# wizardyesterday/RtlSdrDiags

Measured on AMD Instinct MI355X. Metric: IQ MSamples/s through WBFM chain at 1/2/4/8 GPUs; % HBM roofline, higher is better.
Workload: dtype int8/int16 Q15 + f32; 1 GPU; BASELINE configs[1]: WBFM, 1 channel, 2^28-sample synthetic IQ; channels_per_gpu=1, log2_samples_per_channel=28, kernels=streaming pipelines

## Files before the change

rtlsdrdiags_amd/csrc/iqd_stream.hip:

```cpp
#include <hip/hip_runtime.h>

#include "iqd_kernels.h"
#include "iqd_stream.h"
#include "iqd_wbfm.h"
#include "iqd_mfma.h"
#include "iqd_stream_fix.h"
#include "iqd_taps.h"

namespace iqd {

#define ST_STORE16(P, A, B, C, D) (*(u32x4 *)(P) = u32x4{A, B, C, D})


typedef __attribute__((address_space(3))) const uint32_t lds_cu32;
__device__ __forceinline__ uint32_t st_table_read(uint32_t byte_offset) { return *(lds_cu32 *)(uintptr_t)byte_offset; }

#ifndef IQD_ST_WAITSTAT
#define IQD_ST_WAITSTAT 0
#endif

#ifndef IQD_ST_SLEEP_P
#define IQD_ST_SLEEP_P 6
#endif
#ifndef IQD_ST_SLEEP_I
#define IQD_ST_SLEEP_I 10
#endif
#ifndef IQD_ST_SLEEP_A
#define IQD_ST_SLEEP_A 10
#endif
#define ST_TAP(WHICH, Q) (uint32_t)taps::STREAM_TAPS.WHICH[Q]
#ifndef IQD_ST_TRACE
#define IQD_ST_TRACE 0
#endif
#if IQD_ST_TRACE
#define ST_TRACE(st, wave, piece, k) do { if (blockIdx.x == 5 && lane == 0 && (piece) < 256) (st)[64 + (((wave) * 256 + (int)(piece)) * 4 + (k))] = (unsigned long long)clock64(); } while (0)
#else
#define ST_TRACE(st, wave, piece, k) do { } while (0)
#endif
#ifndef IQD_ST_TIMING
#define IQD_ST_TIMING 0
#endif
#if IQD_ST_TIMING
#define ST_T(var) const long long var = clock64()
__device__ __forceinline__ int st_simd_id() { return (__builtin_amdgcn_s_getreg((4 << 0) | (4 << 6) | (1 << 11)) ) & 3; }
#else
#define ST_T(var) do { } while (0)
#endif

template <int ROT, bool MAG, bool EPOCHS, bool GATED, bool BYGROUP = false>
__device__ __forceinline__ void st_p_wave(const ChainLaunch &a, const StreamArgs &sa, uint8_t *lds, uint32_t *sync,
                                          int pw, int lane, uint32_t &pc)
{
    const int cg = pw / ST_RINGS, ring = pw % ST_RINGS;
    if (ring >= (int)sa.rings) return;
    const uint32_t wg_segs = 64u * sa.rings;
    const int g = lane >> 4, c = lane & 15;
    const uint32_t row = (uint32_t)(16 * cg + c);
    uint8_t *ring_base = lds + ST_TABLE_BYTES + ring * (ST_RING_SLOTS * ST_SLOT_BYTES);
    const uint32_t *full = sync + ring * 8;
    asm volatile("" : "+v"(full));
    const uint32_t *consumed = full + 4;
    const uint32_t wr_off = st_slot_off(row, (uint32_t)g);
    const int src_lane4 = ((lane - 16) & 63) << 2;

    v4i A[8];
#pragma unroll
    for (int m = 0; m < 8; m++) A[m] = ((const v4i *)(BYGROUP ? sa.amat3[1 - ROT] : sa.amat))[m * 64 + lane];
    v4i cbias = {WB_BIAS, WB_BIAS, WB_BIAS, WB_BIAS};
    const v4i czero = {0, 0, 0, 0};
    asm volatile("" : "+v"(cbias));
    uint32_t zero = 0;
    asm volatile("" : "+v"(zero));

    const int n_pieces = (ST_HALO + (int)a.tile_len) >> 5;
    uint64_t inv_2pi = 0x3e22f9843e22f984ull;
    asm volatile("" : "+s"(inv_2pi));
    for (uint32_t round = 0; round < sa.rounds; round++) {
        if ((round * chain_wgs(a) + chain_wg(a)) * wg_segs >= st_id_count(sa)) break;
        const uint32_t sid = (round * chain_wgs(a) + chain_wg(a)) * wg_segs + ring * 64 + row;
        int rot_of_id = ROT;
        const StSeg sg = BYGROUP ? st_segment_of(a, sa, sid, rot_of_id) : st_segment(a, sid, sa.n_segments);
        if (BYGROUP && __builtin_amdgcn_readfirstlane(rot_of_id) != ROT) continue;
        const ChanParams &p = a.params[sg.ech];
        const uint8_t *iq_ch = a.iq + (size_t)sg.ch * a.ch_stride_bytes;
        const uint8_t *tail = a.tails + ((size_t)sg.ech * FAM_COUNT + FAM_WBFM) * TAIL_BYTES + TAIL_BYTES;
        const int32_t vmax = sg.vlen - 8;
        const float kneg = -p.wbfm_k;
        const GainEpochList *ep = &a.epochs[sg.ech].wbfm;
        const bool ep_reach = EPOCHS && ep->since[0] < (uint32_t)TAIL && (int64_t)sg.v0 - ST_HALO - 32 < -(int64_t)ep->since[0];
        const bool ep_any = EPOCHS && __any(ep_reach);
        const int32_t mlim = MAG && sg.valid ? sg.tlen : INT32_MIN;
        uint32_t macc = 0;
        const uint32_t mblk0 = (uint32_t)sg.v0 / a.block_samples;
        uint32_t minblk = (uint32_t)sg.v0 - mblk0 * a.block_samples;
        uint32_t *mag_at = MAG ? a.mag_sums + (size_t)sg.ch * a.n_blocks + mblk0 : nullptr;
        uint32_t gm16 = 0;

        const int32_t vlane = sg.v0 + 8 * g;
        const uint8_t *base_iq = iq_ch + 2 * (int64_t)vlane, *base_tail = tail + 2 * (int64_t)vlane;
        const int32_t pos_max = vmax - vlane;
        const uint32_t *blk_list = GATED ? a.blk_lists + (size_t)sg.ch * a.n_blocks : nullptr;
        int32_t gb_v0 = 0, gb_v1 = 0;
        const uint8_t *gb_base = iq_ch;
        auto piece_address = [&](int pos) -> const uint8_t * {
            const int32_t pc = pos < pos_max ? pos : pos_max;
            if (!GATED) {
                const uint8_t *base = pc < -vlane ? base_tail : base_iq;
                return base + 2 * (int64_t)pc;
            }
            const int32_t vv = vlane + pc;
            if (vv >= 0 && (vv >= gb_v1 || vv < gb_v0)) {
                const uint32_t blk = (uint32_t)vv / a.block_samples;
                gb_v0 = (int32_t)(blk * a.block_samples);
                gb_v1 = gb_v0 + (int32_t)a.block_samples;
                gb_base = iq_ch + 2 * ((int64_t)blk_list[blk] * a.block_samples - (int64_t)gb_v0);
            }
            return vv < 0 ? base_tail + 2 * (int64_t)pc : gb_base + 2 * (int64_t)vv;
        };
        const int32_t pos_last = pos_max & ~31;
        const bool from_tail = sg.v0 == 0;
        const uint8_t *nxt = piece_address(-ST_HALO + 32 * ST_AHEAD);
        uint4 prev = st_front<ROT>(*(const uint4 *)piece_address(-ST_HALO - 32), zero);
        v4u raw[ST_AHEAD];
#pragma unroll
        for (int j = 0; j < ST_AHEAD; j++) raw[j] = gload16_untracked(piece_address(-ST_HALO + 32 * j));
        float last_prev;
        {
            const v4i bn = v4i{(int)prev.x, (int)prev.y, (int)prev.z, (int)prev.w};
            const v4i ilo = __builtin_amdgcn_mfma_i32_16x16x64_i8(A[0], bn, cbias, 0, 0, 0);
            const v4i ihi = __builtin_amdgcn_mfma_i32_16x16x64_i8(A[1], bn, czero, 0, 0, 0);
            const v4i qlo = __builtin_amdgcn_mfma_i32_16x16x64_i8(A[2], bn, cbias, 0, 0, 0);
            const v4i qhi = __builtin_amdgcn_mfma_i32_16x16x64_i8(A[3], bn, czero, 0, 0, 0);
            const uint32_t ti = (uint32_t)ilo[3] + ((uint32_t)ihi[3] << 8), tq = (uint32_t)qlo[3] + ((uint32_t)qhi[3] << 8);
            asm volatile("" :: "v"(ilo), "v"(ihi), "v"(qlo), "v"(qhi), "v"(ti), "v"(tq));
            uint32_t rr;
            asm("v_msad_u8 %0, %1, %2, 0" : "=v"(rr) : "v"(tq), "s"(0x00800000u));
            const uint32_t t = st_table_read(rr * (uint32_t)(ST_ROW_FLOATS * 4) + (bfe(ti, 16, 8) << 2));
            last_prev = u2f((t & 0x7fffffffu) | ((tq << 8) & 0x80000000u));
        }
        uint32_t n_sleeps = 0;
#if IQD_ST_TIMING
        long long tt[4] = {0, 0, 0, 0};
#endif
        auto do_piece = [&](const int q, const int j, const uint4 &prev, uint4 &cur) __attribute__((always_inline)) {
            const int pos = -ST_HALO + 32 * q;
            ST_TRACE(a.stamps, pw + 3, q, 0);
            ST_T(t0);
            gload_wait<ST_AHEAD - 1>(raw[j]);
            ST_T(t1);
            const uint4 raw_cur = as_uint4(raw[j]);
            cur = st_front<ROT>(raw_cur, zero);
            const v4i bs = v4i{(int)(lane < 32 ? cur.x : prev.x), (int)(lane < 32 ? cur.y : prev.y),
                               (int)(lane < 32 ? cur.z : prev.z), (int)(lane < 32 ? cur.w : prev.w)};
            const v4i bn = v4i{(int)cur.x, (int)cur.y, (int)cur.z, (int)cur.w};
            v4i acc[2][4];
            acc[0][0] = __builtin_amdgcn_mfma_i32_16x16x64_i8(A[4], bs, cbias, 0, 0, 0);
            acc[0][1] = __builtin_amdgcn_mfma_i32_16x16x64_i8(A[5], bs, czero, 0, 0, 0);
            acc[0][2] = __builtin_amdgcn_mfma_i32_16x16x64_i8(A[6], bs, cbias, 0, 0, 0);
            acc[0][3] = __builtin_amdgcn_mfma_i32_16x16x64_i8(A[7], bs, czero, 0, 0, 0);
            acc[1][0] = __builtin_amdgcn_mfma_i32_16x16x64_i8(A[0], bn, cbias, 0, 0, 0);
            acc[1][1] = __builtin_amdgcn_mfma_i32_16x16x64_i8(A[1], bn, czero, 0, 0, 0);
            acc[1][2] = __builtin_amdgcn_mfma_i32_16x16x64_i8(A[2], bn, cbias, 0, 0, 0);
            acc[1][3] = __builtin_amdgcn_mfma_i32_16x16x64_i8(A[3], bn, czero, 0, 0, 0);
            uint32_t traw[2][4], tqs[2][4];
#pragma unroll
            for (int half = 0; half < 2; half++) {
#pragma unroll
                for (int r = 0; r < 4; r++) {
                    const uint32_t ti = (uint32_t)acc[half][0][r] + ((uint32_t)acc[half][1][r] << 8);
                    const uint32_t tq = (uint32_t)acc[half][2][r] + ((uint32_t)acc[half][3][r] << 8);
                    uint32_t rr;
                    asm("v_msad_u8 %0, %1, %2, 0" : "=v"(rr) : "v"(tq), "s"(0x00800000u));
                    const uint32_t x4 = bfe(ti, 16, 8) << 2;
                    uint32_t addr;
                    asm("v_mad_u32_u24 %0, %1, %2, %3" : "=v"(addr) : "v"(rr), "s"((uint32_t)(ST_ROW_FLOATS * 4)), "v"(x4));
                    traw[half][r] = st_table_read(addr);
                    tqs[half][r] = tq;
                }
            }
            uint32_t seen = lds_load_relaxed(consumed);
            if (MAG && pos >= 0) gm16 = st_mag_raw_chunk(raw_cur, gm16);
            if (GATED) {
                raw[j] = gload16_untracked(piece_address(pos + 32 * ST_AHEAD));
            } else {
                raw[j] = gload16_untracked(nxt);
                nxt += pos + 32 * ST_AHEAD < pos_last ? 64 : 0;
            }
            float u[2][4];
#pragma unroll
            for (int half = 0; half < 2; half++) {
                const int wpos = pos + 16 * half;
                float th[4];
#pragma unroll
                for (int r = 0; r < 4; r++) {
                    uint32_t bits;
                    asm("v_bfi_b32 %0, %1, %2, %3" : "=v"(bits) : "s"(0x7fffffffu), "v"(traw[half][r]), "v"(tqs[half][r] << 8));
                    th[r] = u2f(bits);
                }
                const float give = g == 3 ? last_prev : th[3];
                const float before = u2f((uint32_t)__builtin_amdgcn_ds_bpermute(src_lane4, (int)f2u(give)));
                last_prev = th[3];
                float kk = kneg;
                if (EPOCHS && ep_any && ep_reach) kk = -epoch_gain_search(ep, p.wbfm_k, sg.v0 + wpos);
#pragma unroll
                for (int r = 0; r < 4; r += 2) {
                    v2f d = {th[r] - (r == 0 ? before : th[r - 1]), th[r + 1] - th[r]};
                    v2f m = pk_mul_s(d, inv_2pi);
                    m.x = __builtin_rintf(m.x);
                    m.y = __builtin_rintf(m.y);
                    d = __builtin_elementwise_fma(-m, v2f{6.28318548202514648f, 6.28318548202514648f}, d);
                    d = __builtin_elementwise_fma(-m, v2f{-1.74845553146951715e-7f, -1.74845553146951715e-7f}, d);
                    const v2f v = d * v2f{kk, kk};
                    const v2f w = v2f{sa.b0, sa.b0} * v;
                    u[half][r] = w.x;
                    u[half][r + 1] = w.y;
                }
            }
            ST_T(t2);
            ST_TRACE(a.stamps, pw + 3, q, 1);
            while ((int32_t)(seen + (uint32_t)(ST_DEPTH - 1) - pc) < 0) {
                __builtin_amdgcn_s_sleep(IQD_ST_SLEEP_P);
                seen = lds_load_relaxed(consumed);
                if (IQD_ST_WAITSTAT) n_sleeps++;
            }
            ST_T(t3);
            ST_TRACE(a.stamps, pw + 3, q, 2);
            __builtin_amdgcn_fence(__ATOMIC_ACQUIRE, "workgroup");
            uint8_t *const slot = ring_base + (ST_DEPTH > 1 ? (pc & (uint32_t)(ST_DEPTH - 1)) * (2 * ST_SLOT_BYTES) : 0u) + wr_off;
            *(u32x4 *)slot = u32x4{f2u(u[0][0]), f2u(u[0][1]), f2u(u[0][2]), f2u(u[0][3])};
            *(u32x4 *)(slot + ST_SLOT_BYTES) = u32x4{f2u(u[1][0]), f2u(u[1][1]), f2u(u[1][2]), f2u(u[1][3])};
            __builtin_amdgcn_fence(__ATOMIC_RELEASE, "workgroup");
            lds_signal(ST_DEPTH > 1 ? full + (pc & (uint32_t)(ST_DEPTH - 1)) : full);
            ST_TRACE(a.stamps, pw + 3, q, 3);
            pc++;
#if IQD_ST_TIMING
            { ST_T(t4); tt[0] += t1 - t0; tt[1] += t2 - t1; tt[2] += t3 - t2; tt[3] += t4 - t3; }
#endif
        };
        uint4 other;
        for (int q = 0; q < n_pieces; q += ST_AHEAD) {
#pragma unroll
            for (int j = 0; j < ST_AHEAD; j += 2) {
                do_piece(q + j, j, prev, other);
                do_piece(q + j + 1, j + 1, other, prev);
            }
            const int gpos = -ST_HALO + 32 * q;
            if (!GATED && gpos + 64 * ST_AHEAD == 0)
                nxt = from_tail ? a.iq + (size_t)sg.ch * a.ch_stride_bytes + 16 * g : nxt;
            if (MAG && gpos >= 0) {
                const uint32_t m = (gm16 & 0xffffu) + (gm16 >> 16);
                gm16 = 0;
                macc += gpos < mlim ? m : 0u;
                minblk += 32 * ST_AHEAD;
                if (minblk >= a.block_samples) {
                    if (macc) atomicAdd(mag_at, macc);
                    macc = 0;
                    mag_at++;
                    minblk -= a.block_samples;
                }
            }
        }
#pragma unroll
        for (int j = 0; j < ST_AHEAD; j++) gload_wait<0>(raw[j]);
        if (MAG && macc) atomicAdd(mag_at, macc);
        if (IQD_ST_WAITSTAT && lane == 0) {
            atomicAdd(&a.stamps[0], (unsigned long long)n_sleeps);
            atomicAdd(&a.stamps[2], (unsigned long long)n_pieces);
        }
#if IQD_ST_TIMING
        if (lane == 0) {
            atomicAdd(&a.stamps[16 + pw], (unsigned long long)tt[1]);
            atomicAdd(&a.stamps[32 + pw], (unsigned long long)tt[2]);
            atomicAdd(&a.stamps[48 + pw], (unsigned long long)(tt[0] + tt[3]));
        }
#endif
    }
}

struct StIir {
    float y, up;
    uint32_t wlast[2];
    uint32_t wq0[2];
    uint32_t y1h[4];
    uint32_t y2lo;
    uint32_t n_sleeps;
    int ring;
    unsigned long long *stamps;
#if IQD_ST_TIMING
    long long t_wait, t_seen, t_to_consumed;
#endif
};

__device__ __forceinline__ int st_iir_window(const StreamArgs &sa, StIir &s, const float (&u)[16], int c14, int c15)
{
    uint32_t wq[10];
    float y = s.y, up = s.up;
    const float a1 = sa.a1;
#pragma unroll
    for (int k = 0; k < 8; k++) {
        IQD_IIR_STEP(u[2 * k])
        const float y_even = y;
        IQD_IIR_STEP(u[2 * k + 1])
        wq[2 + k] = cast_pack_i16_bounded(y_even, y);
    }
    s.y = y;
    s.up = up;
    wq[0] = s.wlast[0];
    wq[1] = s.wlast[1];
    s.wlast[0] = wq[8];
    s.wlast[1] = wq[9];
    s.wq0[0] = wq[2];
    s.wq0[1] = wq[3];
    uint32_t y1[4];
#pragma unroll
    for (int o = 0; o < 4; o++) {
        int acc = dot2_from(wq[2 * o], sa.d1p2[0], c15);
        acc = dot2(wq[2 * o + 1], ST_TAP(d1p2, 1), acc);
        acc = dot2(wq[2 * o + 2], ST_TAP(d1p2, 2), acc);
        acc = dot2(wq[2 * o + 3], ST_TAP(d1p2, 3), acc);
        y1[o] = (uint32_t)acc;
    }
    const uint32_t d[6] = {s.y1h[0], s.y1h[1], s.y1h[2], s.y1h[3], pack_hi16(y1[0], y1[1]), pack_hi16(y1[2], y1[3])};
    int acc = dot2_from(d[5], sa.p12p[0], c14);
#pragma unroll
    for (int q = 1; q < 6; q++) acc = dot2(d[5 - q], ST_TAP(p12p, q), acc);
    s.y1h[0] = d[2];
    s.y1h[1] = d[3];
    s.y1h[2] = d[4];
    s.y1h[3] = d[5];
    return acc >> 15;
}

struct StIirSeg {
    StSeg sg;
    int32_t back;
    float cy_y, cy_u;
    int32_t rec_pos;
    WbfmRecord rec;
    StHist *hist;
    int c14, c15;
};

__device__ __forceinline__ bool st_ring_is_fast(uint32_t valid, int32_t back, int32_t tlen, uint32_t tile_len, bool keeps_restart)
{
    return __all(!valid || (back < 0 && tlen == (int32_t)tile_len && !keeps_restart)) != 0;
}

struct StY2Ring {
    uint8_t *lane_slot0;
    const uint32_t *full, *consumed;
};
__device__ __forceinline__ StY2Ring st_y2_ring(uint8_t *lds, uint32_t *sync, int ring, int lane)
{
    return StY2Ring{lds + ST_Y2_OFF + ring * ST_Y2_RING_BYTES + lane * 4, sync + ring * 8 + ST_SYNC_Y2_FULL, sync + ring * 8 + ST_SYNC_Y2_CONSUMED};
}

__device__ __forceinline__ void st_iir_marks(const ChainLaunch &a, StIirSeg &q, StIir &s, int pos, int rec_pos_uniform)
{
    if (q.back >= 0) {
        if (pos == -q.back) { s.y = q.cy_y; s.up = q.cy_u; }
        else if (pos < -q.back) { s.y = 0.f; s.up = 0.f; }
    } else if (pos == 0) {
        q.rec.y_in = s.y;
    }
    if (pos == q.rec_pos) {
        if (q.sg.valid & 2u) {
            q.hist->pad[0] = f2u(s.y);
            q.hist->pad[1] = f2u(s.up);
        } else {
            q.rec.y_out = s.y;
            q.rec.u_out = s.up;
        }
    }
    if ((q.sg.valid & 2u) && pos == rec_pos_uniform) { q.rec.y_out = s.y; q.rec.u_out = s.up; }
    if (pos == q.sg.tlen) {
        q.rec.y_end = s.y;
        q.rec.u_end = s.up;
        if (q.sg.valid) {
            ST_STORE16(q.hist->y1_last, s.y1h[0], s.y1h[1], s.y1h[2], s.y1h[3]);
            *(u32x2 *)q.hist->w_last = u32x2{s.wlast[0], s.wlast[1]};
        }
    }
}

template <bool FAST>
__device__ __forceinline__ void st_iir_piece(const ChainLaunch &a, const StreamArgs &sa, uint8_t *ring_base, const uint32_t *full, uint32_t *consumed,
                                             uint32_t &wg, const StY2Ring &y2r, uint32_t &yk, StIirSeg &q, StIir &s, int pos, uint32_t rd_off0,
                                             uint32_t rd_swz, int lane, int rec_pos_uniform)
{
    uint32_t y2_seen = 0;
#pragma unroll
    for (int half = 0; half < 2; half++) {
        const int wpos = pos + 16 * half;
        if (half == 0) {
            const uint32_t target = 4u * (wg / (uint32_t)ST_DEPTH + 1u);
            const uint32_t *const fullp = ST_DEPTH > 1 ? full + (wg & (uint32_t)(ST_DEPTH - 1)) : full;
            ST_T(tw0);
            while ((int32_t)(lds_load_relaxed(fullp) - target) < 0) {
                __builtin_amdgcn_s_sleep(IQD_ST_SLEEP_I);
                if (IQD_ST_WAITSTAT) s.n_sleeps++;
            }
#if IQD_ST_TIMING
            { ST_T(tw1); s.t_wait += tw1 - tw0; s.t_seen = tw1; }
#endif
            ST_TRACE(s.stamps, s.ring, wg, 0);
            __builtin_amdgcn_fence(__ATOMIC_ACQUIRE, "workgroup");
        }
        const uint8_t *slot = ring_base + (ST_DEPTH > 1 ? (wg & (uint32_t)(ST_DEPTH - 1)) * (2 * ST_SLOT_BYTES) : 0u) + half * ST_SLOT_BYTES + rd_off0;
        float u[16];
#pragma unroll
        for (int gq = 0; gq < 4; gq++) {
            const u32x4 v = *(const u32x4 *)(slot + (((uint32_t)gq ^ rd_swz) << 4));
            u[4 * gq] = u2f(v.x); u[4 * gq + 1] = u2f(v.y); u[4 * gq + 2] = u2f(v.z); u[4 * gq + 3] = u2f(v.w);
        }
        if (half == 1) {
            y2_seen = lds_load_relaxed(y2r.consumed);
            __builtin_amdgcn_fence(__ATOMIC_RELEASE, "workgroup");
            lds_signal(consumed);
            ST_TRACE(s.stamps, s.ring, wg, 1);
            wg++;
#if IQD_ST_TIMING
            { ST_T(tc); s.t_to_consumed += tc - s.t_seen; }
#endif
        }
        if (!FAST) st_iir_marks(a, q, s, wpos, rec_pos_uniform);
        else if (wpos == rec_pos_uniform) { q.rec.y_out = s.y; q.rec.u_out = s.up; }
        const int y2 = st_iir_window(sa, s, u, q.c14, q.c15);
        if (wpos >= 0 && wpos < 48 && q.sg.valid) {
            if (wpos == 0) ST_STORE16(q.hist->w_first, s.wq0[0], s.wq0[1], s.y1h[2], s.y1h[3]);
            else *(u32x2 *)&q.hist->y1_first[wpos >> 3] = u32x2{s.y1h[2], s.y1h[3]};
        }
        if (half == 0) s.y2lo = (uint32_t)y2;
        else {
            const StY2Piece yp = st_y2_piece(yk, ST_Y2_DEPTH, ST_Y2_EVERY);
            while ((int32_t)(y2_seen - yp.need_consumed) < 0) {
                __builtin_amdgcn_s_sleep(IQD_ST_SLEEP_I);
                y2_seen = lds_load_relaxed(y2r.consumed);
                if (IQD_ST_WAITSTAT) s.n_sleeps++;
            }
            __builtin_amdgcn_fence(__ATOMIC_ACQUIRE, "workgroup");
            *(uint32_t *)(y2r.lane_slot0 + yp.slot * ST_Y2_SLOT_BYTES) = pack_lo16(s.y2lo, (uint32_t)y2);
            __builtin_amdgcn_fence(__ATOMIC_RELEASE, "workgroup");
            if (yp.add_full) lds_signal(y2r.full, yp.add_full);
            yk++;
        }
    }
    ST_TRACE(s.stamps, s.ring, wg - 1, 2);
}

__device__ __forceinline__ void st_iir_lead_in(const StreamArgs &sa, uint8_t *ring_base, const uint32_t *full, uint32_t *consumed,
                                               uint32_t &wg, StIir &s, uint32_t rd_off0, uint32_t rd_swz)
{
    float y = s.y, up = s.up;
    const float a1 = sa.a1;
    for (int piece = 0; piece < ST_HALO / 32; piece++) {
        const uint32_t target = 4u * (wg / (uint32_t)ST_DEPTH + 1u);
        while ((int32_t)(lds_load_relaxed(ST_DEPTH > 1 ? full + (wg & (uint32_t)(ST_DEPTH - 1)) : full) - target) < 0) __builtin_amdgcn_s_sleep(IQD_ST_SLEEP_I);
        __builtin_amdgcn_fence(__ATOMIC_ACQUIRE, "workgroup");
        u32x4 v[8];
#pragma unroll
        for (int half = 0; half < 2; half++)
#pragma unroll
            for (int gq = 0; gq < 4; gq++)
                v[4 * half + gq] = *(const u32x4 *)(ring_base + (ST_DEPTH > 1 ? (wg & (uint32_t)(ST_DEPTH - 1)) * (2 * ST_SLOT_BYTES) : 0u) +
                                                    half * ST_SLOT_BYTES + rd_off0 + (((uint32_t)gq ^ rd_swz) << 4));
        __builtin_amdgcn_fence(__ATOMIC_RELEASE, "workgroup");
        lds_signal(consumed);
        wg++;
#pragma unroll
        for (int k = 0; k < 8; k++) {
            IQD_IIR_STEP(u2f(v[k].x)) IQD_IIR_STEP(u2f(v[k].y)) IQD_IIR_STEP(u2f(v[k].z)) IQD_IIR_STEP(u2f(v[k].w))
        }
    }
    s.y = y;
    s.up = up;
}

__device__ __forceinline__ void st_iir_wave(const ChainLaunch &a, const StreamArgs &sa, uint8_t *lds, uint32_t *sync,
                                            int ring, int lane)
{
    uint8_t *ring_base = lds + ST_TABLE_BYTES + ring * (ST_RING_SLOTS * ST_SLOT_BYTES);
    const uint32_t *full = sync + ring * 8;
    uint32_t *consumed = sync + ring * 8 + 4;
    const StY2Ring y2r = st_y2_ring(lds, sync, ring, lane);
    const uint32_t rd_off0 = (uint32_t)lane * 64u, rd_swz = ((uint32_t)lane >> 2) & 3u;
    const int n_pieces = (ST_HALO + (int)a.tile_len) >> 5;
    if (ring >= (int)sa.rings) return;
    const uint32_t wg_segs = 64u * sa.rings;
    uint32_t wg = 0;
    uint32_t yk = 0;
    for (uint32_t round = 0; round < sa.rounds; round++) {
        if ((round * chain_wgs(a) + chain_wg(a)) * wg_segs >= st_id_count(sa)) break;
        const uint32_t sid = (round * chain_wgs(a) + chain_wg(a)) * wg_segs + ring * 64 + lane;
        StIirSeg q;
        int rot_unused;
        q.sg = st_segment_of(a, sa, sid, rot_unused);
        q.hist = sa.hist + (q.sg.valid ? (size_t)q.sg.li * a.tiles_per_ch + q.sg.tile : 0);
        q.back = -1;
        q.cy_y = q.cy_u = 0.f;
        q.c14 = 1 << 14;
        q.c15 = 1 << 15;
        asm volatile("" : "+v"(q.c14), "+v"(q.c15));
        int32_t carried_back = ST_HALO;
        if (q.sg.tile == 0) {
            const WbfmCarry cy = a.wbfm_carry[q.sg.ech];
            q.back = cy.back;
            q.cy_y = cy.y;
            q.cy_u = cy.u;
            carried_back = cy.back;
        }
        const StRecPlan rp = st_rec_plan(q.sg.valid, q.sg.tile, q.sg.v0, q.sg.tlen, q.sg.vlen, carried_back);
        q.rec_pos = rp.park_pos;
        q.rec.y_in = q.cy_y;
        q.rec.y_out = q.cy_y;
        q.rec.u_out = q.cy_u;
        q.rec.back_out = rp.back_out;
        q.rec.y_end = 0.f;
        q.rec.u_end = 0.f;
        q.rec.pad[0] = q.rec.pad[1] = 0;
        const bool keeps_restart = rp.keeps_restart != 0;
        StIir s;
        s.y = 0.f; s.up = 0.f;
        s.wlast[0] = s.wlast[1] = 0;
        s.wq0[0] = s.wq0[1] = 0;
#pragma unroll
        for (int k = 0; k < 4; k++) s.y1h[k] = 0;
        s.y2lo = 0;
        s.n_sleeps = 0;
        s.ring = ring;
        s.stamps = a.stamps;
#if IQD_ST_TIMING
        s.t_wait = 0;
        s.t_seen = 0;
        s.t_to_consumed = 0;
        const long long t_iir0 = clock64();
#endif
        const bool fast = st_ring_is_fast(q.sg.valid, q.back, q.sg.tlen, a.tile_len, keeps_restart);
        if (keeps_restart) q.sg.valid |= 2u;
        const int rec_pos_uniform = (int)a.tile_len - FORCED_BACK;
        if (fast) {
            st_iir_lead_in(sa, ring_base, full, consumed, wg, s, rd_off0, rd_swz);
            q.rec.y_in = s.y;
            for (int pq = ST_HALO / 32; pq < n_pieces; pq++)
                st_iir_piece<true>(a, sa, ring_base, full, consumed, wg, y2r, yk, q, s, -ST_HALO + 32 * pq, rd_off0, rd_swz, lane, rec_pos_uniform);
        } else {
            for (int pq = 0; pq < n_pieces; pq++)
                st_iir_piece<false>(a, sa, ring_base, full, consumed, wg, y2r, yk, q, s, -ST_HALO + 32 * pq, rd_off0, rd_swz, lane, rec_pos_uniform);
        }
        st_iir_marks(a, q, s, (int)a.tile_len, rec_pos_uniform);
        if (q.sg.valid) {
            WbfmRecord *const r = a.records + (size_t)q.sg.li * a.tiles_per_ch + q.sg.tile;
            if (q.sg.valid & 2u) {
                q.rec.pad[0] = q.hist->pad[0];
                q.rec.pad[1] = q.hist->pad[1];
            } else if (!(q.sg.vlen - q.sg.v0 > q.sg.tlen)) {
                q.rec.pad[0] = WBFM_REC_STREAMED;
            }
            *r = q.rec;
        }
        if (IQD_ST_WAITSTAT && lane == 0) {
            atomicAdd(&a.stamps[1], (unsigned long long)s.n_sleeps);
            atomicAdd(&a.stamps[3], (unsigned long long)n_pieces);
        }
#if IQD_ST_TIMING
        if (lane == 0) {
            atomicAdd(&a.stamps[28 + ring], (unsigned long long)s.t_wait);
            atomicAdd(&a.stamps[44 + ring], (unsigned long long)(clock64() - t_iir0));
            atomicAdd(&a.stamps[60 + ring], (unsigned long long)s.t_to_consumed);
        }
#endif
    }
}

template <int V>
__device__ __forceinline__ int st_audio(const StreamArgs &sa, const uint32_t (&y2p)[24], bool quiet, int c14)
{
    int acc = c14;
    if (quiet) {
        acc = dot2_from(y2p[V + 20], sa.a40p[0], c14);
#pragma unroll
        for (int q = 1; q < 20; q++) acc = dot2(y2p[V + 20 - q], ST_TAP(a40p, q), acc);
    } else {
#pragma unroll
        for (int q = 0; q < 20; q++) {
            acc = clamp_q30(dot2(y2p[V + 20 - q], ST_TAP(a40p, q) & 0xffff0000u, acc));
            acc = clamp_q30(dot2(y2p[V + 20 - q], ST_TAP(a40p, q) & 0x0000ffffu, acc));
        }
    }
    return acc >> 15;
}

struct StAudRing {
    uint32_t y2p[24];
    uint32_t pbuf[2];
    int16_t *pcm;
    uint32_t hidx;
    int32_t tlen;
};

template <int V>
__device__ __forceinline__ uint32_t st_audio_piece(const StreamArgs &sa, const StY2Ring &y2r, uint32_t &ak, StAudRing &r, int &loud, int c14)
{
    const StY2Piece yp = st_y2_piece(ak, ST_Y2_DEPTH, ST_Y2_EVERY);
    while ((int32_t)(lds_load_relaxed(y2r.full) - yp.need_full) < 0) __builtin_amdgcn_s_sleep(IQD_ST_SLEEP_A);
    __builtin_amdgcn_fence(__ATOMIC_ACQUIRE, "workgroup");
    const uint32_t pair = *(const uint32_t *)(y2r.lane_slot0 + yp.slot * ST_Y2_SLOT_BYTES);
    __builtin_amdgcn_fence(__ATOMIC_RELEASE, "workgroup");
    lds_signal(y2r.consumed);
    ak++;
    r.y2p[V + 20] = pair;
    const int lo = (int)(pair << 16) >> 16, hi = (int)pair >> 16;
    const uint32_t mlo = (uint32_t)(lo < 0 ? -lo : lo), mhi = (uint32_t)(hi < 0 ? -hi : hi);
    if (__any(mlo > (uint32_t)AUDIO40_SAFE || mhi > (uint32_t)AUDIO40_SAFE)) loud = 21;
    const uint32_t pcm = (uint32_t)(loud == 0 ? st_audio<V>(sa, r.y2p, true, c14) : st_audio<V>(sa, r.y2p, false, c14));
    if (loud > 0) loud--;
    return pcm;
}

__device__ __forceinline__ void st_audio_quad_done(const StreamArgs &sa, StAudRing &r, int pos, bool wide, uint32_t w0, uint32_t w1)
{
    const bool valid = r.hidx != ~0u;
    if (pos >= 0 && pos < 768 - 96 && valid)
        ST_STORE16(&sa.hist[r.hidx].y2_first[pos >> 5], r.y2p[20], r.y2p[21], r.y2p[22], r.y2p[23]);
    if (!wide) {
        if (valid && pos >= 0 && pos < r.tlen) *(u32x2 *)(r.pcm + (pos >> 5)) = u32x2{w0, w1};
    } else if (((pos >> 7) & 1) == 0) {
        r.pbuf[0] = w0;
        r.pbuf[1] = w1;
    } else if (valid) {
        const int g0 = pos - 128;
        int16_t *dst = r.pcm + (g0 >> 5);
        if (g0 >= 0 && g0 + 256 <= r.tlen) {
            ST_STORE16(dst, r.pbuf[0], r.pbuf[1], w0, w1);
        } else {
            if (g0 >= 0 && g0 < r.tlen) ((u32x2 *)dst)[0] = u32x2{r.pbuf[0], r.pbuf[1]};
            if (pos >= 0 && pos < r.tlen) ((u32x2 *)dst)[1] = u32x2{w0, w1};
        }
    }
#pragma unroll
    for (int k = 0; k < 20; k++) r.y2p[k] = r.y2p[k + 4];
}

__device__ __forceinline__ void st_audio_end_mark(const StreamArgs &sa, const StAudRing &r, int pos)
{
    if (pos == r.tlen && r.hidx != ~0u) {
#pragma unroll
        for (int k = 0; k < 20; k += 4) ST_STORE16(&sa.hist[r.hidx].y2_last[k], r.y2p[k], r.y2p[k + 1], r.y2p[k + 2], r.y2p[k + 3]);
    }
}

static_assert(ST_RINGS == 3, "ST_FOR_RINGS names the rings");
#define ST_FOR_RINGS(...) do { { constexpr int ring = 0; __VA_ARGS__ } { constexpr int ring = 1; __VA_ARGS__ } { constexpr int ring = 2; __VA_ARGS__ } } while (0)

__device__ __forceinline__ int st_audio_ring_start(const ChainLaunch &a, const StreamArgs &sa, uint32_t round, int ring, int lane, StAudRing &r)
{
#pragma unroll
    for (int k = 0; k < 24; k++) r.y2p[k] = 0;
    r.pbuf[0] = r.pbuf[1] = 0;
    const uint32_t sid = (round * chain_wgs(a) + chain_wg(a)) * (64u * sa.rings) + ring * 64 + lane;
    int rot_unused;
    const StSeg sg = st_segment_of(a, sa, sid, rot_unused);
    const int32_t back = sg.tile == 0 ? a.wbfm_carry[sg.ech].back : -1;
    const StRecPlan rp = st_rec_plan(sg.valid, sg.tile, sg.v0, sg.tlen, sg.vlen, sg.tile == 0 ? back : ST_HALO);
    const bool fast = st_ring_is_fast(sg.valid, back, sg.tlen, a.tile_len, rp.keeps_restart != 0);
    r.pcm = a.pcm + (size_t)sg.ch * a.pcm_stride + (sg.v0 >> 5);
    r.hidx = sg.valid ? sg.li * a.tiles_per_ch + sg.tile : ~0u;
    r.tlen = sg.tlen;
    return fast ? ST_HALO / 32 : 0;
}

__device__ __forceinline__ void st_audio_wave(const ChainLaunch &a, const StreamArgs &sa, uint8_t *lds, uint32_t *sync, int lane)
{
    const int n_pieces = (ST_HALO + (int)a.tile_len) >> 5;
    const bool wide = (a.tile_len & 511u) == 0 && (((uintptr_t)a.pcm | (a.pcm_stride * 2)) & 31u) == 0;
    int c14 = 1 << 14;
    asm volatile("" : "+v"(c14));
    StY2Ring y2r[ST_RINGS];
    uint32_t ak[ST_RINGS];
    ST_FOR_RINGS(y2r[ring] = st_y2_ring(lds, sync, ring, lane); ak[ring] = 0;);
    for (uint32_t round = 0; round < sa.rounds; round++) {
        if ((round * chain_wgs(a) + chain_wg(a)) * (64u * sa.rings) >= st_id_count(sa)) break;
        StAudRing r[ST_RINGS];
        int loud[ST_RINGS], pq0[ST_RINGS];
        ST_FOR_RINGS(
            loud[ring] = 0;
            pq0[ring] = n_pieces;
            if (ring < (int)sa.rings) pq0[ring] = st_audio_ring_start(a, sa, round, ring, lane, r[ring]);
        );
        for (int pq = 0; pq < n_pieces; pq += 4) {
            const int pos = -ST_HALO + 32 * pq;
            ST_FOR_RINGS(if (pq >= pq0[ring]) {
                st_audio_end_mark(sa, r[ring], pos);
                const uint32_t p0 = st_audio_piece<0>(sa, y2r[ring], ak[ring], r[ring], loud[ring], c14);
                const uint32_t p1 = st_audio_piece<1>(sa, y2r[ring], ak[ring], r[ring], loud[ring], c14);
                const uint32_t p2 = st_audio_piece<2>(sa, y2r[ring], ak[ring], r[ring], loud[ring], c14);
                const uint32_t p3 = st_audio_piece<3>(sa, y2r[ring], ak[ring], r[ring], loud[ring], c14);
                st_audio_quad_done(sa, r[ring], pos, wide, pack_lo16(p0, p1), pack_lo16(p2, p3));
            });
        }
        ST_FOR_RINGS(if (ring < (int)sa.rings) st_audio_end_mark(sa, r[ring], (int)a.tile_len););
    }
}
#undef ST_FOR_RINGS

template <int ROT, bool MAG, bool EPOCHS, bool GATED>
__device__ __forceinline__ void wbfm_stream_body(const ChainLaunch &a, const StreamArgs &sa, uint8_t *st_lds)
{
    if ((uint32_t)(uintptr_t)(__attribute__((address_space(3))) uint8_t *)st_lds != 0u) __builtin_trap();
    uint32_t *sync = (uint32_t *)(st_lds + ST_SYNC_OFF);
    const int tid = (int)threadIdx.x;
    {
        constexpr int N16 = ST_TABLE_BYTES / 16, TRIPS = (N16 + ST_THREADS - 1) / ST_THREADS;
        uint4 t[TRIPS];
#pragma unroll
        for (int k = 0; k < TRIPS; k++) {
            const int i = tid + k * ST_THREADS;
            t[k] = ((const uint4 *)sa.half_lut)[i < N16 ? i : N16 - 1];
        }
#pragma unroll
        for (int k = 0; k < TRIPS; k++) {
            const int i = tid + k * ST_THREADS;
            if (i < N16) ((uint4 *)st_lds)[i] = t[k];
        }
    }
    if (tid < ST_SYNC_WORDS) sync[tid] = 0;
    __syncthreads();
    const int wave = __builtin_amdgcn_readfirstlane(tid >> 6), lane = tid & 63;
    uint32_t pc = 0;
#if IQD_ST_TIMING
    if (blockIdx.x == 0 && lane == 0) a.stamps[20000 + wave] = (unsigned long long)(st_simd_id() + 1);
#endif
    if (wave < ST_RINGS) st_iir_wave(a, sa, st_lds, sync, wave, lane);
    else if (wave == ST_AUDIO_WAVE) st_audio_wave(a, sa, st_lds, sync, lane);
    else if (ROT != 2) st_p_wave<ROT, MAG, EPOCHS, GATED>(a, sa, st_lds, sync, wave - ST_RINGS, lane, pc);
    else {
        st_p_wave<1, MAG, EPOCHS, GATED, true>(a, sa, st_lds, sync, wave - ST_RINGS, lane, pc);
        st_p_wave<0, MAG, EPOCHS, GATED, true>(a, sa, st_lds, sync, wave - ST_RINGS, lane, pc);
        st_p_wave<-1, MAG, EPOCHS, GATED, true>(a, sa, st_lds, sync, wave - ST_RINGS, lane, pc);
    }
}

#ifndef IQD_STREAM_BODIES_ONLY
template <int ROT, bool MAG, bool EPOCHS, bool GATED>
__global__ __launch_bounds__(ST_THREADS, 4) void wbfm_stream_kernel(const ChainLaunch a, const StreamArgs sa)
{
    extern __shared__ __attribute__((aligned(16))) uint8_t st_lds[];
    wbfm_stream_body<ROT, MAG, EPOCHS, GATED>(a, sa, st_lds);
}
#endif

#ifndef IQD_STREAM_BODIES_ONLY
__global__ __launch_bounds__(FIX_THREADS) void wbfm_stream_fixup_kernel(const ChainLaunch a, const StreamArgs sa)
{
    __shared__ FixLds fl;
    wbfm_stream_fixup_body(a, sa, blockIdx.x, fl);
}

hipError_t launch_wbfm_stream_fixup(const ChainLaunch &a, const StreamArgs &sa, hipStream_t s)
{
    hipLaunchKernelGGL(wbfm_stream_fixup_kernel, dim3((sa.n_segments + FIX_SEGS - 1) / FIX_SEGS), dim3(FIX_THREADS), 0, s, a, sa);
    return hipGetLastError();
}

typedef void (*StKernel)(const ChainLaunch, const StreamArgs);
#define ST_K(R) {{wbfm_stream_kernel<R, false, false, false>, wbfm_stream_kernel<R, false, true, false>}, \
                 {wbfm_stream_kernel<R, true, false, false>, wbfm_stream_kernel<R, true, true, false>},   \
                 {wbfm_stream_kernel<R, false, false, true>, wbfm_stream_kernel<R, false, true, true>}}
static const StKernel st_kernels[4][3][2] = {ST_K(-1), ST_K(0), ST_K(1), ST_K(2)};
#undef ST_K

hipError_t init_wbfm_stream_kernels()
{
    for (int r = 0; r < 4; r++)
        for (int g = 0; g < 6; g++) {
            const hipError_t e = hipFuncSetAttribute((const void *)st_kernels[r][g >> 1][g & 1], hipFuncAttributeMaxDynamicSharedMemorySize, ST_LDS_BYTES);
            if (e != hipSuccess) return e;
        }
    return hipSuccess;
}

hipError_t launch_wbfm_stream(const ChainLaunch &a, const StreamArgs &sa, int rotation, bool mag, bool epochs, uint32_t grid, hipStream_t s)
{
    const int variant = a.vlen_gated ? 2 : (mag ? 1 : 0);
    hipLaunchKernelGGL(st_kernels[sa.grouped ? 3 : rotation < 0 ? 0 : rotation > 0 ? 2 : 1][variant][epochs ? 1 : 0], dim3(grid), dim3(ST_THREADS), ST_LDS_BYTES, s, a, sa);
    return hipGetLastError();
}

#endif

}
```

Before: 849,600 MSamples/s.

## Repack phase-diff pairs, clamp prefetch offset, and split prologue loop

```diff
diff --git a/rtlsdrdiags_amd/csrc/iqd_stream.hip b/rtlsdrdiags_amd/csrc/iqd_stream.hip
--- a/rtlsdrdiags_amd/csrc/iqd_stream.hip
+++ b/rtlsdrdiags_amd/csrc/iqd_stream.hip
@@ -120,6 +120,12 @@
         const int32_t pos_last = pos_max & ~31;
         const bool from_tail = sg.v0 == 0;
         const uint8_t *nxt = piece_address(-ST_HALO + 32 * ST_AHEAD);
+        constexpr int ST_NXT_ORIGIN = -ST_HALO + 32 * ST_AHEAD;
+        auto nxt_room = [&](int32_t from) -> uint32_t {
+            const int64_t room = 2 * ((int64_t)pos_last - from);
+            return room < 0 ? 0u : room > 0x7fffff00 ? 0x7fffff00u : (uint32_t)room;
+        };
+        uint32_t nxt_max = nxt_room(ST_NXT_ORIGIN);
         uint4 prev = st_front<ROT>(*(const uint4 *)piece_address(-ST_HALO - 32), zero);
         v4u raw[ST_AHEAD];
 #pragma unroll
@@ -183,52 +189,51 @@
             if (GATED) {
                 raw[j] = gload16_untracked(piece_address(pos + 32 * ST_AHEAD));
             } else {
-                raw[j] = gload16_untracked(nxt);
-                nxt += pos + 32 * ST_AHEAD < pos_last ? 64 : 0;
-            }
-            float u[2][4];
+                const uint32_t at = (uint32_t)(2 * (pos + 32 * ST_AHEAD - ST_NXT_ORIGIN));
+                raw[j] = gload16_untracked(nxt + (at < nxt_max ? at : nxt_max));
+            }
+            v2f u[2][2];
 #pragma unroll
             for (int half = 0; half < 2; half++) {
                 const int wpos = pos + 16 * half;
-                float th[4];
-#pragma unroll
-                for (int r = 0; r < 4; r++) {
-                    uint32_t bits;
-                    asm("v_bfi_b32 %0, %1, %2, %3" : "=v"(bits) : "s"(0x7fffffffu), "v"(traw[half][r]), "v"(tqs[half][r] << 8));
-                    th[r] = u2f(bits);
-                }
-                const float give = g == 3 ? last_prev : th[3];
+                uint32_t th[4], th1_z;
+#pragma unroll
+                for (int r = 0; r < 4; r++)
+                    asm("v_bfi_b32 %0, %1, %2, %3" : "=v"(th[r]) : "s"(0x7fffffffu), "v"(traw[half][r]), "v"(tqs[half][r] << 8));
+                asm("v_bfi_b32 %0, %1, %2, %3 ; theta1 of the pair Z" : "=v"(th1_z) : "s"(0x7fffffffu), "v"(traw[half][1]), "v"(tqs[half][1] << 8));
+                const float give = g == 3 ? last_prev : u2f(th[3]);
                 const float before = u2f((uint32_t)__builtin_amdgcn_ds_bpermute(src_lane4, (int)f2u(give)));
-                last_prev = th[3];
+                last_prev = u2f(th[3]);
                 float kk = kneg;
                 if (EPOCHS && ep_any && ep_reach) kk = -epoch_gain_search(ep, p.wbfm_k, sg.v0 + wpos);
-#pragma unroll
-                for (int r = 0; r < 4; r += 2) {
-                    v2f d = {th[r] - (r == 0 ? before : th[r - 1]), th[r + 1] - th[r]};
+                const v2f X = {u2f(th[0]), u2f(th[2])}, Y = {before, u2f(th[1])}, Z = {u2f(th1_z), u2f(th[3])};
+#pragma unroll
+                for (int e = 0; e < 2; e++) {
+                    v2f d = e == 0 ? X - Y : Z - X;
                     v2f m = pk_mul_s(d, inv_2pi);
                     m.x = __builtin_rintf(m.x);
                     m.y = __builtin_rintf(m.y);
                     d = __builtin_elementwise_fma(-m, v2f{6.28318548202514648f, 6.28318548202514648f}, d);
                     d = __builtin_elementwise_fma(-m, v2f{-1.74845553146951715e-7f, -1.74845553146951715e-7f}, d);
                     const v2f v = d * v2f{kk, kk};
-                    const v2f w = v2f{sa.b0, sa.b0} * v;
-                    u[half][r] = w.x;
-                    u[half][r + 1] = w.y;
+                    u[half][e] = v2f{sa.b0, sa.b0} * v;
                 }
             }
             ST_T(t2);
             ST_TRACE(a.stamps, pw + 3, q, 1);
+            seen = (uint32_t)__builtin_amdgcn_readfirstlane((int)seen);
             while ((int32_t)(seen + (uint32_t)(ST_DEPTH - 1) - pc) < 0) {
                 __builtin_amdgcn_s_sleep(IQD_ST_SLEEP_P);
                 seen = lds_load_relaxed(consumed);
+                seen = (uint32_t)__builtin_amdgcn_readfirstlane((int)seen);
                 if (IQD_ST_WAITSTAT) n_sleeps++;
             }
             ST_T(t3);
             ST_TRACE(a.stamps, pw + 3, q, 2);
             __builtin_amdgcn_fence(__ATOMIC_ACQUIRE, "workgroup");
             uint8_t *const slot = ring_base + (ST_DEPTH > 1 ? (pc & (uint32_t)(ST_DEPTH - 1)) * (2 * ST_SLOT_BYTES) : 0u) + wr_off;
-            *(u32x4 *)slot = u32x4{f2u(u[0][0]), f2u(u[0][1]), f2u(u[0][2]), f2u(u[0][3])};
-            *(u32x4 *)(slot + ST_SLOT_BYTES) = u32x4{f2u(u[1][0]), f2u(u[1][1]), f2u(u[1][2]), f2u(u[1][3])};
+            *(u32x4 *)slot = u32x4{f2u(u[0][0].x), f2u(u[0][0].y), f2u(u[0][1].x), f2u(u[0][1].y)};
+            *(u32x4 *)(slot + ST_SLOT_BYTES) = u32x4{f2u(u[1][0].x), f2u(u[1][0].y), f2u(u[1][1].x), f2u(u[1][1].y)};
             __builtin_amdgcn_fence(__ATOMIC_RELEASE, "workgroup");
             lds_signal(ST_DEPTH > 1 ? full + (pc & (uint32_t)(ST_DEPTH - 1)) : full);
             ST_TRACE(a.stamps, pw + 3, q, 3);
@@ -238,26 +243,33 @@
 #endif
         };
         uint4 other;
-        for (int q = 0; q < n_pieces; q += ST_AHEAD) {
-#pragma unroll
-            for (int j = 0; j < ST_AHEAD; j += 2) {
-                do_piece(q + j, j, prev, other);
-                do_piece(q + j + 1, j + 1, other, prev);
-            }
-            const int gpos = -ST_HALO + 32 * q;
-            if (!GATED && gpos + 64 * ST_AHEAD == 0)
-                nxt = from_tail ? a.iq + (size_t)sg.ch * a.ch_stride_bytes + 16 * g : nxt;
-            if (MAG && gpos >= 0) {
-                const uint32_t m = (gm16 & 0xffffu) + (gm16 >> 16);
-                gm16 = 0;
-                macc += gpos < mlim ? m : 0u;
-                minblk += 32 * ST_AHEAD;
-                if (minblk >= a.block_samples) {
-                    if (macc) atomicAdd(mag_at, macc);
-                    macc = 0;
-                    mag_at++;
-                    minblk -= a.block_samples;
+        const int q_samples = !GATED ? ST_HALO / 32 - ST_AHEAD : n_pieces;
+        int q = 0;
+#pragma unroll 1
+        for (int q_end = q_samples; q < n_pieces; q_end = n_pieces) {
+            for (; q < q_end; q += ST_AHEAD) {
+#pragma unroll
+                for (int j = 0; j < ST_AHEAD; j += 2) {
+                    do_piece(q + j, j, prev, other);
+                    do_piece(q + j + 1, j + 1, other, prev);
                 }
+                const int gpos = -ST_HALO + 32 * q;
+                if (MAG && gpos >= 0) {
+                    const uint32_t m = (gm16 & 0xffffu) + (gm16 >> 16);
+                    gm16 = 0;
+                    macc += gpos < mlim ? m : 0u;
+                    minblk += 32 * ST_AHEAD;
+                    if (minblk >= a.block_samples) {
+                        if (macc) atomicAdd(mag_at, macc);
+                        macc = 0;
+                        mag_at++;
+                        minblk -= a.block_samples;
+                    }
+                }
+            }
+            if (!GATED && q == q_samples && from_tail) {
+                nxt = (const uint8_t *)((uintptr_t)(a.iq + (size_t)sg.ch * a.ch_stride_bytes + 16 * g) + (intptr_t)(2 * ST_NXT_ORIGIN));
+                nxt_max = nxt_room(0) + (uint32_t)(-2 * ST_NXT_ORIGIN);
             }
         }
 #pragma unroll
@@ -411,7 +423,7 @@
 #pragma unroll
         for (int gq = 0; gq < 4; gq++) {
             const u32x4 v = *(const u32x4 *)(slot + (((uint32_t)gq ^ rd_swz) << 4));
-            u[4 * gq] = u2f(v.x); u[4 * gq + 1] = u2f(v.y); u[4 * gq + 2] = u2f(v.z); u[4 * gq + 3] = u2f(v.w);
+            u[4 * gq] = u2f(v.x); u[4 * gq + 2] = u2f(v.y); u[4 * gq + 1] = u2f(v.z); u[4 * gq + 3] = u2f(v.w);
         }
         if (half == 1) {
             y2_seen = lds_load_relaxed(y2r.consumed);
@@ -469,7 +481,7 @@
         wg++;
 #pragma unroll
         for (int k = 0; k < 8; k++) {
-            IQD_IIR_STEP(u2f(v[k].x)) IQD_IIR_STEP(u2f(v[k].y)) IQD_IIR_STEP(u2f(v[k].z)) IQD_IIR_STEP(u2f(v[k].w))
+            IQD_IIR_STEP(u2f(v[k].x)) IQD_IIR_STEP(u2f(v[k].z)) IQD_IIR_STEP(u2f(v[k].y)) IQD_IIR_STEP(u2f(v[k].w))
         }
     }
     s.y = y;
```

Measured after the change: 859,000 MSamples/s, median of 6. 1.01x the previous value.
